# meudnaes/VoronoiRT

Measured on AMD Instinct MI355X. Metric: formal-solve cell-updates/sec, higher is better.
Workload: dtype f64

## Files before the change

### include/voronoirt.h

```cpp
#ifndef VORONOIRT_H
#define VORONOIRT_H

#include <stdint.h>

#ifdef __cplusplus
extern "C" {
#endif

#define VRT_OK 0
#define VRT_EINVAL (-1)
#define VRT_EGRID (-2)
#define VRT_ENODEVICE (-3)
#define VRT_ENOMEM (-4)
#define VRT_EIO (-5)

typedef struct vrt_grid vrt_grid;
typedef struct vrt_plan vrt_plan;

#define VRT_ALPHA_SITE 0
#define VRT_ALPHA_SITE_LAM 1
#define VRT_ALPHA_ANGLE_SITE_LAM 2
#define VRT_ALPHA_ANGLE_NATIVE 3
#define VRT_ALPHA_SITE_LAM_NATIVE 4

// ... 73 lines not shown
                                     double lambda0, double c0, const double *d_doppler_width, const double *d_gamma,
                                     double sigma_bb_const, const double *sigma_bf1, const double *sigma_bf2,
                                     const double *d_temperature, const double *d_lte_populations, double hc_over_kB,
                                     double pref_ij, double pref_ji, const double *d_C, const double *d_atom_density,
                                     double *d_R, double *d_populations, void *stream);
int vrt_lambda_update_native_dev_f32(vrt_plan *p, int64_t nlam, const float *dJ_up, const float *dJ_down,
                                     const float *dB_up, const double *deps, float *dS_up, float *dS_down,
                                     double *max_rel_change, void *stream);
int vrt_rates_populations_native_dev_f32(vrt_plan *p, int64_t nlam, const double *lambda, const int64_t blocks[6],
                                         const float *dJ_up, const float *dJ_down, const double *planck2,
                                         double lambda0, double c0, const double *d_doppler_width, const double *d_gamma,
                                         double sigma_bb_const, const double *sigma_bf1, const double *sigma_bf2,
                                         const double *d_temperature, const double *d_lte_populations, double hc_over_kB,
                                         double pref_ij, double pref_ji, const double *d_C, const double *d_atom_density,
                                         double *d_R, double *d_populations, void *stream);

int vrt_plan_execute_dev_f32(vrt_plan *p, int64_t nlam, int64_t ld, const float *dS,
                             const float *dalpha, int alpha_mode, const float *dI0_up,
                             const float *dI0_down, const double *weights_host, float *dJ,
                             float *dI_out, void *stream);
int vrt_plan_last_sweep_timing(const vrt_plan *p, double *ms, int64_t *launches);
int vrt_plan_patch_layout(const vrt_plan *p, int64_t *out);
int vrt_patch_dispatch_map(int order, int nrow, int nsplit, int lg_siblings, int64_t nred, int steps, int64_t *dims, int32_t *blocks);
int vrt_plan_patch_timeline(vrt_plan *p, int64_t cap_launches, int64_t cap_blocks, int64_t *launches, uint64_t *stamps, int64_t *counts);
int vrt_plan_check(vrt_plan *p);
int vrt_plan_last_path(const vrt_plan *p);
int vrt_plan_set_option(vrt_plan *p, const char *name, const char *value);
int vrt_grid_set_option(vrt_grid *g, const char *name, const char *value);

typedef struct vrt_schedule vrt_schedule;
int vrt_schedule_build(const vrt_grid *g, int dir, const int64_t *up, int n_sweeps, vrt_schedule **out);
int64_t vrt_schedule_num_nodes(const vrt_schedule *s);
int64_t vrt_schedule_num_levels(const vrt_schedule *s);
int vrt_schedule_get(const vrt_schedule *s, int64_t *site, int32_t *zflags, int64_t *level_off);
void vrt_schedule_destroy(vrt_schedule *s);
int vrt_layer_schedule(const vrt_grid *g, int dir, const int64_t *up, int n_sweeps, uint32_t *vis,
                       int32_t *nlev, int64_t *n_visits);
int vrt_layer_sorted_slots(const vrt_grid *g, int dir, const uint32_t *vis, int64_t *store, int64_t *self);

typedef struct vrt_patch_schedule vrt_patch_schedule;
int vrt_patch_schedule_build(const vrt_grid *g, int dir, const int64_t *up, int n_sweeps, int own_target,
                             int entry_cap, vrt_patch_schedule **out, int64_t counts[6]);
int vrt_patch_schedule_get(const vrt_patch_schedule *s, int32_t *layer_patch_off, int32_t *patch_own_lo,
                           int32_t *patch_own_cnt, int32_t *patch_nlev, int64_t *patch_ent_off,
                           int32_t *entry_pos, uint32_t *entry_vis, uint32_t *entry_loc);
int vrt_patch_schedule_get_deps(const vrt_patch_schedule *s, int64_t *dep_off, int32_t *dep_list);
// ... 248 lines not shown
```

### voronoirt_amd/_lib.py

```python
from __future__ import annotations

import ctypes
import os

HERE = os.path.dirname(os.path.abspath(__file__))
LIB_PATH = os.path.join(HERE, "libvrt_hip.so")
if os.environ.get("VRT_LIB_PATH"):
    LIB_PATH = os.environ["VRT_LIB_PATH"]

c_i64 = ctypes.c_int64
c_dbl = ctypes.c_double
p_i64 = ctypes.POINTER(ctypes.c_int64)
p_i32 = ctypes.POINTER(ctypes.c_int32)
p_dbl = ctypes.POINTER(ctypes.c_double)
p_int = ctypes.POINTER(ctypes.c_int)
vp = ctypes.c_void_p

VRT_OK, VRT_EINVAL, VRT_EGRID, VRT_ENODEVICE, VRT_ENOMEM, VRT_EIO = 0, -1, -2, -3, -4, -5
ALPHA_SITE, ALPHA_SITE_LAM, ALPHA_ANGLE_SITE_LAM, ALPHA_ANGLE_NATIVE, ALPHA_SITE_LAM_NATIVE = 0, 1, 2, 3, 4
METRIC_EUCLIDEAN, METRIC_PERIODIC_XY = 0, 1
RASTER_NEAREST, RASTER_INV_DIST2 = 1, 2
REG_FORMS = ("solve<256>", "solve<1024>", "xy_march_lds<1>", "xy_march_lds<2>", "xy_march_lds<4>", "xy_march_lds<0>",
             "xy_march_mem")
REG_FORM_KERNEL_MASK, REG_FORM_YZ_ROW_MARCH, REG_FORM_XZ_ROW_MARCH = 0xff, 0x100, 0x200
# ... 76 lines not shown
    "vrt_lambda_storage": (ctypes.c_int, [vp]),
    "vrt_lambda_iterate": (ctypes.c_int, [vp, p_dbl]),
    "vrt_lambda_get": (ctypes.c_int, [vp, p_dbl, p_dbl, p_dbl, p_dbl, p_dbl]),
    "vrt_lambda_destroy": (None, [vp]),
    "vrt_multi_create": (ctypes.c_int, [ctypes.c_int, p_int, c_i64, p_dbl, p_i64, c_i64, p_dbl, c_i64, p_dbl, p_int,
                                        ctypes.c_int, ctypes.POINTER(vp)]),
    "vrt_multi_execute": (ctypes.c_int, [vp, c_i64, c_i64, p_dbl, p_dbl, ctypes.c_int, p_dbl, p_dbl, p_dbl, p_dbl]),
    "vrt_multi_set_shard": (ctypes.c_int, [vp, ctypes.c_char_p]),
    "vrt_multi_last_shard": (ctypes.c_int, [vp]),
    "vrt_multi_uses_rccl": (ctypes.c_int, [vp]),
    "vrt_multi_destroy": (None, [vp]),
    "vrt_multi_execute_line": (ctypes.c_int, [vp, c_i64, c_i64, p_dbl, c_dbl, c_dbl, p_dbl, p_dbl, p_dbl, p_dbl, p_dbl, p_dbl,
                                              p_dbl, p_dbl, p_dbl, p_dbl]),
    "vrt_multi_lambda_create": (ctypes.c_int, [vp, ctypes.POINTER(LineCaseStruct), p_dbl, ctypes.POINTER(vp)]),
    "vrt_multi_lambda_iterate": (ctypes.c_int, [vp, p_dbl]),
    "vrt_multi_lambda_get": (ctypes.c_int, [vp, p_dbl, p_dbl, p_dbl, p_dbl, p_dbl]),
    "vrt_multi_lambda_destroy": (None, [vp]),
    "vrt_rates_populations_dev": (ctypes.c_int, [vp, c_i64, c_i64, p_dbl, p_i64, vp, p_dbl, c_dbl, c_dbl, vp, vp,
                                                 c_dbl, p_dbl, p_dbl, vp, vp, c_dbl, c_dbl, c_dbl, vp, vp, vp,
                                                 vp, vp]),
    "vrt_plan_last_sweep_timing": (ctypes.c_int, [vp, p_dbl, p_i64]),
    "vrt_plan_patch_layout": (ctypes.c_int, [vp, p_i64]),
    "vrt_patch_dispatch_map": (ctypes.c_int, [ctypes.c_int, ctypes.c_int, ctypes.c_int, ctypes.c_int, c_i64, ctypes.c_int, p_i64, p_i32]),
    "vrt_plan_patch_timeline": (ctypes.c_int, [vp, c_i64, c_i64, p_i64, ctypes.POINTER(ctypes.c_uint64), p_i64]),
    "vrt_plan_last_path": (ctypes.c_int, [vp]),
    "vrt_plan_set_option": (ctypes.c_int, [vp, ctypes.c_char_p, ctypes.c_char_p]),
    "vrt_grid_set_option": (ctypes.c_int, [vp, ctypes.c_char_p, ctypes.c_char_p]),
    "vrt_schedule_build": (ctypes.c_int, [vp, ctypes.c_int, p_i64, ctypes.c_int,
                                          ctypes.POINTER(vp)]),
    "vrt_schedule_num_nodes": (c_i64, [vp]),
    "vrt_schedule_num_levels": (c_i64, [vp]),
    "vrt_schedule_get": (ctypes.c_int, [vp, p_i64, p_i32, p_i64]),
    "vrt_schedule_destroy": (None, [vp]),
    "vrt_layer_schedule": (ctypes.c_int, [vp, ctypes.c_int, p_i64, ctypes.c_int,
                                          ctypes.POINTER(ctypes.c_uint32), p_i32, p_i64]),
    "vrt_layer_sorted_slots": (ctypes.c_int, [vp, ctypes.c_int, ctypes.POINTER(ctypes.c_uint32), p_i64, p_i64]),
    "vrt_patch_schedule_build": (ctypes.c_int, [vp, ctypes.c_int, p_i64, ctypes.c_int, ctypes.c_int, ctypes.c_int,
                                                ctypes.POINTER(vp), p_i64]),
    "vrt_patch_schedule_get": (ctypes.c_int, [vp, p_i32, p_i32, p_i32, p_i32, p_i64, p_i32,
                                              ctypes.POINTER(ctypes.c_uint32), ctypes.POINTER(ctypes.c_uint32)]),
    "vrt_patch_schedule_get_deps": (ctypes.c_int, [vp, p_i64, p_i32]),
    "vrt_patch_schedule_get_layers": (ctypes.c_int, [vp, ctypes.POINTER(ctypes.c_uint32), p_i32, p_i64]),
    "vrt_patch_schedule_destroy": (None, [vp]),
    "vrt_lambda_update_dev": (ctypes.c_int, [vp, c_i64, c_i64, vp, vp, vp, vp, vp, p_dbl, vp]),
    "vrt_short_characteristics": (ctypes.c_int, [c_i64, c_i64, c_i64, p_dbl, p_dbl, p_dbl, c_i64, p_dbl,
                                                 p_int, p_dbl, c_i64, p_dbl, c_i64, p_dbl, ctypes.c_int,
# ... 138 lines not shown
```

### voronoirt_amd/csrc/vrt_api.cpp

```cpp
#include <algorithm>
#include <atomic>
#include <chrono>
#include <cmath>
#include <cstdio>
#include <cstdlib>
#include <cstring>
#include <memory>
#include <new>
#include <thread>

#include "vrt_internal.h"

namespace vrt {

static thread_local std::string g_err;

void set_error(const std::string &msg) { g_err = msg; }
int fail(int code, const std::string &msg)
{
    g_err = msg;
    return code;
}

int check_source(const double *S, int64_t count)
// ... 6 lines not shown
int check_state_pointers(const void *session, const double *S, const double *populations)
{
    if (!session) return fail(VRT_EINVAL, "NULL session");
    if (!S && !populations) return fail(VRT_EINVAL, "S and populations are both NULL: nothing to set");
    return VRT_OK;
}

int check_state(int64_t n, int64_t nlam, const double *S, const double *populations)
{
    if (S)
        if (int rc = check_source(S, n * nlam)) return rc;
    if (populations)
        for (int64_t i = 0; i < 3 * n; i++)
            if (!std::isfinite(populations[i]) || !(populations[i] >= 0.0))
                return fail(VRT_EINVAL, "the populations must be finite and >= 0 everywhere");
    return VRT_OK;
}

void tuning_from_env(Tuning &t)
{
    static const char *names[] = {"VRT_PATH", "VRT_STEP_K", "VRT_STEP_SINGLE", "VRT_STEP_PAIRS", "VRT_STEP_XCD",
                                  "VRT_STEP_STREAMS", "VRT_STEP_LEVEL_MAP", "VRT_STEP_GROUP_DIR", "VRT_TILE_WIDE",
                                  "VRT_TILE_PRE", "VRT_PATCH_K", "VRT_PATCH_NT", "VRT_PATCH_OWN",
                                  "VRT_PATCH_Q", "VRT_PATCH_TARGET", "VRT_PATCH_SPLIT", "VRT_PATCH_ORDER", "VRT_PATCH_TIMELINE", "VRT_PAIR_BLOCK", "VRT_PATCH_QUAD", "VRT_PATCH_LEAN", "VRT_PATCH_CHAIN", "VRT_CHAIN_PAIRS", "VRT_CHAIN_SPIN", "VRT_CHAIN_DATAFLAG", "VRT_CHAIN_STATIC", "VRT_LAMBDA_NATIVE", "VRT_DEBUG_FLAGS", "VRT_DEBUG_SKIP_LEVELS",
                                  "VRT_TILE_DEBUG"};
    for (const char *nm : names) {
        const char *e = std::getenv(nm);
        if (e && *e && tuning_set(t, nm, e, false) != VRT_OK) {
            static std::mutex mu;
            static std::vector<std::string> said;
            std::lock_guard<std::mutex> lock(mu);
            if (std::find(said.begin(), said.end(), std::string(nm)) == said.end()) {
                said.push_back(nm);
                std::fprintf(stderr, "[libvrt_hip] ignoring %s=%s: %s\n", nm, e, g_err.c_str());
            }
        }
    }
}

int tuning_set(Tuning &t, const char *name, const char *value, bool created)
{
    if (!name || !value) return fail(VRT_EINVAL, "NULL option name or value");
    const std::string nm(name), v(value);
    if (nm == "VRT_PATH") {
        static const char *paths[] = {"auto", "levels", "tiles", "steps", "patches"};
        for (int i = 0; i < 5; i++)
            if (v == paths[i]) { t.path = i; return VRT_OK; }
        if (v.empty()) { t.path = 0; return VRT_OK; }
        return fail(VRT_EINVAL, "VRT_PATH must be auto, levels, tiles, steps or patches");
    }
    char *end = nullptr;
    const long x = std::strtol(value, &end, 10);
    if (end == value || *end != 0) return fail(VRT_EINVAL, "option " + nm + " needs an integer value");
    struct { const char *name; int *field; long lo, hi; bool creation_only; } tab[] = {
        {"VRT_STEP_K", &t.step_K, 0, 18, false}, {"VRT_STEP_SINGLE", &t.step_single, 0, 1, false},
        {"VRT_STEP_PAIRS", &t.step_pairs, 0, 64, false}, {"VRT_STEP_XCD", &t.step_xcd, 0, 2, false},
        {"VRT_STEP_STREAMS", &t.step_streams, 1, 4, false}, {"VRT_STEP_LEVEL_MAP", &t.step_level_map, 0, 1, false},
        {"VRT_STEP_GROUP_DIR", &t.step_group_dir, 0, 1, false}, {"VRT_TILE_WIDE", &t.tile_wide, 0, 1, false},
        {"VRT_TILE_PRE", &t.tile_pre, 0, 1, false},
        {"VRT_PATCH_K", &t.patch_K, 1, 8, true}, {"VRT_PATCH_NT", &t.patch_NT, 64, 1024, true},
        {"VRT_PATCH_OWN", &t.patch_own, 0, 65535, true}, {"VRT_PATCH_Q", &t.patch_Q, 1, 4, false},
        {"VRT_PATCH_TARGET", &t.patch_target, 0, 1 << 20, false}, {"VRT_PATCH_SPLIT", &t.patch_split, 0, 4096, false}, {"VRT_PATCH_ORDER", &t.patch_order, 0, 1, false},
        {"VRT_PATCH_TIMELINE", &t.patch_timeline, 0, 1, false}, {"VRT_PAIR_BLOCK", &t.pair_block, 1, 16, true},
        {"VRT_PATCH_QUAD", &t.patch_quad, 0, 1, true}, {"VRT_PATCH_LEAN", &t.patch_lean, 0, 1, false},
        {"VRT_PATCH_CHAIN", &t.patch_chain, 0, 2, false}, {"VRT_CHAIN_PAIRS", &t.chain_pairs, 1, 256, false},
        {"VRT_CHAIN_SPIN", &t.chain_spin, 1, 1 << 20, false}, {"VRT_CHAIN_DATAFLAG", &t.chain_dataflag, 0, 2, false},
        {"VRT_LAMBDA_NATIVE", &t.lambda_native, 0, 1, false}, {"VRT_CHAIN_STATIC", &t.chain_static, 0, 1, false}, {"VRT_DEBUG_FLAGS", &t.debug_flags, 0, 1 << 20, false},
        {"VRT_DEBUG_SKIP_LEVELS", &t.debug_skip_levels, 0, 1, false}, {"VRT_TILE_DEBUG", &t.tile_debug, 0, 1, false},
    };
    for (auto &o : tab)
        if (nm == o.name) {
            if (o.creation_only && created)
                return fail(VRT_EINVAL, "option " + nm + " shapes what plan creation builds: preset it in the environment");
            if (x < o.lo || x > o.hi) return fail(VRT_EINVAL, "option " + nm + " out of range");
            *o.field = (int)x;
            return VRT_OK;
        }
    return fail(VRT_EINVAL, "unknown option " + nm);
}

int use_device(int device)
{
    if (device < 0)
        return fail(VRT_ENODEVICE, "host-only grid handle (device < 0): no compute without a HIP device");
    int cnt = 0;
    hipError_t e = hipGetDeviceCount(&cnt);
    if (e != hipSuccess || cnt <= 0)
        return fail(VRT_ENODEVICE, "no HIP device available (libvrt_hip has no CPU fallback)");
    if (device < 0 || device >= cnt) return fail(VRT_EINVAL, "device ordinal out of range");
    VRT_HIP_TRY(hipSetDevice(device));
    (void)hipGetLastError();
    return VRT_OK;
// ... 1168 lines not shown
    const int maxL = p->tile_max_layers;
    int64_t fewest = 0;
    if (p->patch_ok && !p->h_patch_first.empty()) {
        fewest = INT64_MAX;
        for (int a = 0; a < p->A; a++)
            for (int layer = 2; layer <= maxL; layer++) {
                const int32_t *first = p->h_patch_first.data() + (size_t)a * (size_t)(maxL + 2);
                fewest = std::min<int64_t>(fewest, first[layer + 1] - first[layer]);
            }
        if (fewest == INT64_MAX) fewest = 0;
    }
    out[0] = p->patch_ok ? p->n_patches : 0;
    out[1] = fewest;
    out[2] = p->patch_work_off.empty() ? 0 : p->patch_work_off.back();
    out[3] = p->patch_work_padding;
    return VRT_OK;
}

int vrt_patch_dispatch_map(int order, int nrow, int nsplit, int lg_siblings, int64_t nred, int steps, int64_t *dims, int32_t *blocks)
{
    return guarded([&] { return patch_dispatch_map(order, nrow, nsplit, lg_siblings, nred, steps, dims, blocks); });
}

int vrt_plan_patch_timeline(vrt_plan *p, int64_t cap_launches, int64_t cap_blocks, int64_t *launches, uint64_t *stamps, int64_t *counts)
{
    if (!p || !launches || !stamps || !counts) return fail(VRT_EINVAL, "NULL plan or output");
    return guarded([&] {
        std::lock_guard<std::mutex> lock(p->mu);
        if (int rc = use_device(p->device)) return rc;
        return patch_timeline_read(p, cap_launches, cap_blocks, launches, stamps, counts);
    });
}

int vrt_plan_last_sweep_timing(const vrt_plan *p, double *ms, int64_t *launches)
{
    if (!p) return fail(VRT_EINVAL, "NULL plan");
    if (!p->ev_valid) return fail(VRT_EINVAL, "no execute has run on this plan yet");
    return guarded([&] {
        VRT_HIP_TRY(hipEventSynchronize(p->ev1));
        float t = 0.f;
        VRT_HIP_TRY(hipEventElapsedTime(&t, p->ev0, p->ev1));
        if (ms) *ms = (double)t;
        if (launches) *launches = p->last_launches;
        return patch_chain_check(const_cast<vrt_plan *>(p));
    });
}
// ... 304 lines not shown
```

### voronoirt_amd/csrc/vrt_device.h

```cpp
#pragma once

#include <hip/hip_runtime.h>

#include "vrt_internal.h"
#include "vrt_weights.h"

namespace vrt {

#ifdef VRT_DIAG
constexpr bool kDiag = true;
#else
constexpr bool kDiag = false;
#endif

constexpr uint32_t kNoSlot = 0xFFFFu;

__host__ __device__ __forceinline__ void pair_block_at(int q, int npair, int lgB, int &k0, int &lw)
{
    const int full = npair >> lgB << lgB;
    if (q < full) { k0 = q >> lgB << lgB; lw = lgB; return; }
    int k = full;
    const int r = npair - full;
    for (int bit = lgB - 1; bit >= 0; bit--)
        if (r & (1 << bit)) {
// ... 115 lines not shown
};

__device__ __forceinline__ double2 ld2(const double2 *base, unsigned idx)
{
    return *reinterpret_cast<const double2 *>(reinterpret_cast<const char *>(base) + ((size_t)idx << 4));
}
__device__ __forceinline__ double2 ld2(const float2 *base, unsigned idx)
{
    return to_d2(*reinterpret_cast<const float2 *>(reinterpret_cast<const char *>(base) + ((size_t)idx << 3)));
}

__device__ __forceinline__ void upwind_term(double r, double w, double a_c, double a_u, double S_c,
                                            double S_u, double I_u, bool early, bool inl, double &t,
                                            double &g, bool cheap = false)
{
    double ca, cb, ce;
    if (cheap) { ca = a_c; cb = a_u; ce = r; }
    else
    lin_weights(r * (a_c + a_u) / 2.0, ca, cb, ce);
    t = early ? ((ce * I_u + ca * S_u) + cb * S_c) * w : (ca * S_u + cb * S_c) * w;
    g = inl ? ce * w : 0.0;
}

struct PatchReduce {
    int nred = 0;
    int nblk[2] = {0, 0};
    int lo[2] = {0, 0}, hi[2] = {0, 0};
    int count[2] = {0, 0};
    int ppb = 4;
    void *Jd[2] = {nullptr, nullptr};
    double w[kMaxAngles];
    int32_t angles[2][kMaxAngles];
};


}
```

### voronoirt_amd/csrc/vrt_internal.h

```cpp
#pragma once

#include <hip/hip_runtime.h>

#include <algorithm>
#include <cstdint>
#include <memory>
#include <mutex>
#include <new>
#include <string>
#include <thread>
#include <vector>

#include "voronoirt.h"

namespace vrt {

void set_error(const std::string &msg);
int fail(int code, const std::string &msg);

int check_source(const double *S, int64_t count);
int check_state_pointers(const void *session, const double *S, const double *populations);
int check_state(int64_t n, int64_t nlam, const double *S, const double *populations);

#define VRT_HIP_TRY(expr)                                                                  \
// ... 155 lines not shown
        } catch (...) {
            threw[(size_t)t] = 1;
        }
    };
    std::vector<std::thread> pool;
    try {
        pool.reserve((size_t)std::max(count, 1));
    } catch (...) {
    }
    for (int t = 0; t < count; t++) {
        try {
            pool.emplace_back(guarded, t);
        } catch (...) {
            guarded(t);
        }
    }
    for (auto &th : pool) th.join();
    for (int t = 0; t < count; t++)
        if (threw[(size_t)t]) return false;
    return true;
}

constexpr int kMaxAngles = 64;
constexpr int64_t kMaxGuess = 70;
constexpr int32_t kNoUpwind = -1;

struct Direction {
    std::vector<int32_t> layer_of;
    std::vector<int64_t> perm;
    std::vector<int64_t> reduced;
    int64_t n1 = 0;
    DevBuf<int32_t> d_order;
    DevBuf<int32_t> d_rank;
    DevBuf<int32_t> d_lay;
    std::vector<int32_t> store;
    DevBuf<int32_t> d_store;
    DevBuf<int32_t> d_srank;
};

struct PlanCacheEntry;

struct CopyLane {
    Stream st;
    HostBuf<char> pin[2];
    Event ev[2];
};
// ... 4 lines not shown
    int step_K = 0;
    int step_single = 0;
    int step_pairs = 0;
    int step_xcd = 2;
    int step_streams = 2;
    int step_level_map = 1;
    int step_group_dir = 1;
    int tile_wide = 1;
    int tile_pre = 1;
    int patch_K = 1, patch_NT = 512;
    int patch_own = 0;
    int patch_Q = 1;
    int pair_block = 1;
    int patch_quad = 1;
    int patch_lean = 1;
    int patch_chain = 2;
    int chain_pairs = 9;
    int chain_spin = 2048;
    int chain_dataflag = 2;
    int patch_split = 0;
    int patch_target = 0;
    int patch_order = 1;
    int patch_timeline = 0;
    int chain_static = 1;
    int lambda_native = 1;
    int debug_flags = 0, debug_skip_levels = 0, tile_debug = 0;
};
void tuning_from_env(Tuning &t);
int tuning_set(Tuning &t, const char *name, const char *value, bool created);

struct ExecArgs {
    int64_t nlam = 0, ld = 0;
    const void *S = nullptr;
    const void *S_nat[2] = {nullptr, nullptr};
    const void *alpha = nullptr;
    int alpha_mode = 0;
    const void *I0[2] = {nullptr, nullptr};
    const double *weights = nullptr;
    void *J = nullptr;
    void *J_nat[2] = {nullptr, nullptr};
    void *I_out = nullptr;
    bool native = false;
    bool f32 = false;
    hipStream_t st = nullptr;
    bool wants_J() const { return native ? J_nat[0] != nullptr : J != nullptr; }
};
// ... 310 lines not shown
}
int alpha_to_native(vrt_plan *p, int64_t nlam, int64_t ld, const void *dalpha, void *out, hipStream_t st, bool f32);
int native_planes_ok(const vrt_plan *p, bool f32 = false);
int planes_to_native_f32(vrt_plan *p, int64_t nlam, int64_t ld, const float *din, float *out_up, float *out_down, hipStream_t st);
int plane_from_native_f32(vrt_plan *p, int dir_index, int64_t nlam, int64_t ld, const float *din, float *dout, hipStream_t st);
int J_from_native_f32(vrt_plan *p, int64_t nlam, int64_t ld, const float *dJ_up, const float *dJ_down, float *dJ, hipStream_t st);
int planes_to_native(vrt_plan *p, int64_t nlam, int64_t ld, const double *din, double *out_up, double *out_down, hipStream_t st);
int plane_from_native(vrt_plan *p, int dir_index, int64_t nlam, int64_t ld, const double *din, double *dout, hipStream_t st);
int J_from_native(vrt_plan *p, int64_t nlam, int64_t ld, const double *dJ_up, const double *dJ_down, double *dJ, hipStream_t st);
int execute_layers(vrt_plan *p, const ExecArgs &x, int path);
int64_t steps_max_layer(bool f32);

struct TileArgs;
struct PatchReduce;
bool patch_shape_exists(int K, int Q, int NT);
int launch_patch_entries(vrt_plan *p, int a, int64_t first, int64_t count);
int ensure_patch_work(vrt_plan *p, int G, const std::vector<int32_t> &group_angles, const std::vector<int> &group_off);
int launch_patch_layer(vrt_plan *p, const TileArgs &ta, int npair, int layer, int group, int Q, hipStream_t st,
                       bool f32, const PatchReduce *reduce);
constexpr int kPatchTimelineRec = 12;
void patch_timeline_begin(vrt_plan *p);
int patch_timeline_read(vrt_plan *p, int64_t cap_launches, int64_t cap_blocks, int64_t *launches, uint64_t *stamps, int64_t *counts);
int patch_dispatch_map(int order, int nrow, int nsplit, int lg_siblings, int64_t nred, int steps, int64_t *dims, int32_t *blocks);
bool patch_chain_possible(const vrt_plan *p, int npair, bool f32);
bool patch_chain_dataflag(const vrt_plan *p, int npair, bool f32);
int launch_patch_chain(vrt_plan *p, const TileArgs &ta, int npair, hipStream_t st, bool f32, const PatchReduce *reduce,
                       bool dataflag, bool ctrl_zeroed = false);
int chain_ctrl_words();
int patch_chain_check(vrt_plan *p);

struct NgRange {
    int64_t dense = 0, tail = 0, tstride = 1;
};
struct NgState {
    int order = 0, start = 0, period = 0;
    DevBuf<double> hist[3];
    unsigned have = 0;
    DevBuf<double> d_ws;
    int last_applied = 0;
    double last_sums[5] = {0, 0, 0, 0, 0}, last_coeffs[2] = {0, 0};
};
inline NgRange ng_S_range(int64_t n, int64_t nlam, bool sweep_order)
{
    NgRange rg;
    if (sweep_order) { rg.dense = (nlam / 2) * 2 * n; rg.tail = nlam & 1 ? n : 0; rg.tstride = 2; }
    else { rg.dense = (n * nlam) & ~(int64_t)1; rg.tail = (n * nlam) & 1; rg.tstride = 1; }
// ... 54 lines not shown
```

### voronoirt_amd/csrc/vrt_patch.hip

```cpp
#include <hip/hip_runtime.h>

#include <algorithm>
#include <cmath>
#include <cstdio>
#include <cstdlib>
#include <cstring>
#include <type_traits>

#include "vrt_device.h"
#include "vrt_internal.h"

namespace vrt {

enum : int {
    kDiagNoLevels = 1, kDiagCentreGathers = 2, kDiagNoWeights = 4, kDiagNoStores = 8, kDiagNoGatherI = 16, kDiagNoGatherAlpha = 32,
    kDiagNoGatherS = 64, kDiagNoReduce = 128, kDiagNoWait = 256, kDiagPlainLoadI = 512, kDiagPlainStoreI = 1024, kDiagNoPairLoop = 2048,
    kDiagDirectTable = 4096,
};
__host__ __device__ __forceinline__ constexpr bool diag(int dbg, int flag) { return kDiag && (dbg & flag) != 0; }

struct PatchArgs {
    TileArgs ta;
    int npair;
    int layer;
    int ngrp;
    int nrow;
    int order;
    int prow;
    unsigned row_rcp;
    int nsplit, Q;
    int sbase, srem;
    int lgB;
    int stride;
    int cap;
    int quad;
    int lean;
    int dbg_ent0, dbg_ent_stride, dbg_ent_last;
    int dbg;
    unsigned long long *tl;
    PatchReduce red;
    const int4 *wrec;
    const int32_t *e_pos, *e_u1, *e_u2;
    const uint32_t *e_vis, *e_loc;
    const double *e_w1, *e_w2, *e_r1, *e_r2;
};

__global__ void __launch_bounds__(256)
k_patch_entries(int64_t count, const int32_t *__restrict__ e_pos, const int32_t *__restrict__ t_u1,
                const int32_t *__restrict__ t_u2, const double *__restrict__ t_w1, const double *__restrict__ t_w2,
                const double *__restrict__ t_r1, const double *__restrict__ t_r2, int32_t *__restrict__ e_u1,
                int32_t *__restrict__ e_u2, double *__restrict__ e_w1, double *__restrict__ e_w2,
                double *__restrict__ e_r1, double *__restrict__ e_r2)
{
    const int64_t e = (int64_t)blockIdx.x * blockDim.x + threadIdx.x;
    if (e >= count) return;
    const int p = e_pos[e];
    e_u1[e] = t_u1[p]; e_u2[e] = t_u2[p];
    e_w1[e] = t_w1[p]; e_w2[e] = t_w2[p];
    e_r1[e] = t_r1[p]; e_r2[e] = t_r2[p];
}

int launch_patch_entries(vrt_plan *p, int a, int64_t first, int64_t count)
{
// ... 97 lines not shown
    {
        if (kDiag && pa.tl) {
            slot = pa.tl + 3 * ((size_t)blockIdx.y * gridDim.x + blockIdx.x);
            t0 = wall_clock64();
        }
    }
    __device__ __forceinline__ void steps(const PatchArgs &pa, int b0, int b1)
    {
        if (kDiag) share = (unsigned long long)((b1 - b0 + pa.Q - 1) / pa.Q);
    }
    __device__ __forceinline__ void reduces()
    {
        if (kDiag) share = 1ull << 32;
    }
    __device__ __forceinline__ ~BlockStamp()
    {
        if (kDiag && slot && threadIdx.x == 0) {
            slot[0] = t0;
            slot[1] = wall_clock64();
            slot[2] = share;
        }
    }
};
template <typename T, int NT>
__device__ __forceinline__ void patch_reduce_role(const PatchArgs &pa)
{
    typedef typename Pair<T>::type T2;
    const TileArgs &ta = pa.ta;
    const int tid = threadIdx.x;
    int b = reduce_block_index(pa), r = 0;
    if (b >= pa.red.nblk[0]) { b -= pa.red.nblk[0]; r = 1; }
    if (b >= pa.red.nblk[r]) return;
    if (diag(pa.dbg, kDiagNoReduce)) return;
    const int len = pa.red.hi[r] - pa.red.lo[r];
    const int per = NT * pa.red.ppb;
    const int nblock = pair_block_count(pa.npair, pa.lgB);
    int k0 = 0, lw = 0;
    for (int k = 0; k < nblock; k++) {
        pair_block_of(k, pa.npair, pa.lgB, k0, lw);
        const int cnt = (int)((((int64_t)len << lw) + per - 1) / per);
        if (b < cnt) break;
        b -= cnt;
    }
    const int64_t nn = ta.n;
    const size_t run = (size_t)len << lw;
    const size_t base = (size_t)k0 * (size_t)nn + ((size_t)pa.red.lo[r] << lw);
    T2 *Jd = reinterpret_cast<T2 *>(pa.red.Jd[r]);
    const T2 *I0 = reinterpret_cast<const T2 *>(ta.I);
    const size_t plane = (size_t)pa.npair * (size_t)nn;
    if (pa.red.ppb == 4) {
        const size_t f0 = (size_t)b * 4 * NT + tid;
        const unsigned left = f0 < run ? (unsigned)min((size_t)(run - f0 + NT - 1) / NT, (size_t)4) : 0u;
        const size_t e0 = base + (left ? f0 : 0);
        double ax[4], ay[4];
#pragma unroll
        for (int i = 0; i < 4; i++) { ax[i] = 0.0; ay[i] = 0.0; }
        for (int j = 0; j < pa.red.count[r]; j++) {
            const int a = pa.red.angles[r][j];
            const T2 *Ia = I0 + (size_t)a * plane + e0;
            double2 v[4];
#pragma unroll
            for (int i = 0; i < 4; i++) v[i] = to_d2(Ia[(unsigned)i < left ? i * NT : 0]);
#pragma unroll
            for (int i = 0; i < 4; i++) {
                ax[i] += pa.red.w[a] * v[i].x;
                ay[i] += pa.red.w[a] * v[i].y;
            }
        }
#pragma unroll
        for (int i = 0; i < 4; i++)
            if ((unsigned)i < left) Jd[e0 + (size_t)i * NT] = from_d2<T>(make_double2(ax[i], ay[i]));
        return;
    }
    for (int i = 0; i < pa.red.ppb; i++) {
        const size_t f = ((size_t)b * pa.red.ppb + i) * NT + tid;
        if (f >= run) break;
        const size_t e = base + f;
        double ax = 0.0, ay = 0.0;
        for (int j = 0; j < pa.red.count[r]; j++) {
            const int a = pa.red.angles[r][j];
            const double2 v = to_d2(I0[(size_t)a * plane + e]);
            ax += pa.red.w[a] * v.x;
            ay += pa.red.w[a] * v.y;
        }
        Jd[e] = from_d2<T>(make_double2(ax, ay));
    }
}

#ifdef VRT_PATCH_WPE
#define VRT_WPE_ATTR __attribute__((amdgpu_waves_per_eu(VRT_PATCH_WPE, VRT_PATCH_WPE)))
#else
#define VRT_WPE_ATTR
#endif
template <typename T, int AM, int K, int Q, int NT>
__global__ void __launch_bounds__(NT) VRT_WPE_ATTR
k_patch_solve(PatchArgs pa)
{
    typedef typename Pair<T>::type T2;
    extern __shared__ __attribute__((aligned(16))) double2 ptile[];
    const TileArgs &ta = pa.ta;
    const int tid = threadIdx.x;
    BlockStamp stamp(pa);
    if (reduce_block_index(pa) >= 0) {
        stamp.reduces();
        patch_reduce_role<T, NT>(pa);
        return;
    }
    const PatchBlock blk = patch_block(pa, pa.lgB);
    const int x = blk.lane, sj = blk.row;
// ... 746 lines not shown
    __syncthreads();
    quad_pairs<AM, NT, false>(pair_io<AM>(pa, it.d), it, tab, ptile);
}


struct ChainDev {
    TileArgs ta;
    int npair, nsplit, cap;
    const int32_t *e_pos, *e_u1, *e_u2;
    const uint32_t *e_vis, *e_loc;
    const double *e_w1, *e_w2, *e_r1, *e_r2;
    PatchReduce red;
    const int4 *items;
    int q_off[9];
    const int32_t *deps;
    uint32_t *progress;
    uint32_t *ctrl;
    uint32_t *host_status;
    int64_t n_patches;
    uint32_t spin_limit;
    int static_items;
    int dbg;
};

__device__ __forceinline__ const uint32_t *chain_abort_word(const uint32_t *cd_words)
{
    return reinterpret_cast<const ChainDev *>(cd_words)->ctrl + kChainAbortWord;
}

__device__ __forceinline__ int cd_int(const int *p) { return __builtin_amdgcn_readfirstlane(*p); }
template <typename P>
__device__ __forceinline__ P *cd_ptr(P *const *p) { return uniform_ptr(*p); }

__device__ __forceinline__ void chain_wait_slow(const int32_t *s_dep, int step)
{
    const int lane = (int)(threadIdx.x & 63u);
    const uint32_t *ctl = reinterpret_cast<const uint32_t *>(s_dep - kCtlWords);
    const ChainDev *cd = reinterpret_cast<const ChainDev *>(((uint64_t)ctl[kCtlArgsHi] << 32) | (uint64_t)ctl[kCtlArgsLo]);
    uint32_t *abort_word = cd->ctrl + kChainAbortWord;
    const uint32_t *progress = chain_progress(ctl);
    const uint32_t target = ctl[kCtlBase] + (uint32_t)step, limit = cd->spin_limit;
    const int ndep = (int)ctl[kCtlNdep];
    for (int c0 = 0; c0 < ndep; c0 += 64) {
        const int j = c0 + lane;
        const int dep = j < 64 + kChainDepLds ? s_dep[j] : (j < ndep ? (cd->deps + ctl[kCtlDepOff])[j] : (int)ctl[kCtlSelf]);
        const uint32_t *w = progress + dep;
// ... 271 lines not shown
            const size_t base = work.size();
            work.resize(base + slots * 8 * 2, make_int4(0, 0, 0, 0));
            p->patch_work_padding += (int64_t)(slots * 8 - m);
            for (int x = 0; x < 8; x++) {
                const size_t b0 = m * (size_t)x / 8, b1 = m * (size_t)(x + 1) / 8;
                for (size_t t = b0; t < b1; t++) {
                    const int32_t q = items[t].second;
                    const int2 r2 = p->h_patch_rec2[(size_t)q];
                    const int d = p->dir_of_active[(size_t)r2.y] > 0 ? 0 : 1;
                    const Direction &dir = d == 0 ? p->g->up : p->g->down;
                    const size_t slot = base + 2 * ((t - b0) * 8 + (size_t)x);
                    work[slot] = p->h_patch_rec[(size_t)q];
                    work[slot + 1] = make_int4(r2.x, r2.y | (d << 16), (int)(dir.reduced[(size_t)layer - 1] - 1), (int)(dir.reduced[(size_t)layer] - 1));
                }
            }
        }
    p->patch_work_off.back() = (int64_t)(work.size() / 2);
    if (int rc = p->d_patch_work.alloc(work.size())) return rc;
    VRT_HIP_TRY(hipMemcpy(p->d_patch_work, work.data(), sizeof(int4) * work.size(), hipMemcpyHostToDevice));
    p->patch_work_groups = G;
    return VRT_OK;
}

static void size_reduce(PatchReduce &red, int npair, int lgB, int NT)
{
    red.nred = 0;
    int64_t total = 0;
    for (int r = 0; r < 2; r++)
        if (red.count[r] > 0 && red.Jd[r]) total += (int64_t)std::max(0, red.hi[r] - red.lo[r]) * npair;
    red.ppb = total <= (int64_t)NT * 1024 ? 1 : 4;
    const int64_t per = (int64_t)NT * red.ppb;
    const int nblock = pair_block_count(npair, lgB);
    for (int r = 0; r < 2; r++) {
        const int64_t len = red.hi[r] - red.lo[r];
        red.nblk[r] = 0;
        if (len > 0 && red.count[r] > 0 && red.Jd[r])
            for (int k = 0; k < nblock; k++) {
                int k0, lw;
                pair_block_of(k, npair, lgB, k0, lw);
                red.nblk[r] += (int)(((len << lw) + per - 1) / per);
            }
        red.nred += red.nblk[r];
    }
    red.nred = (red.nred + 7) / 8 * 8;
}

int launch_patch_layer(vrt_plan *p, const TileArgs &ta, int npair, int layer, int group, int Q, hipStream_t st,
                       bool f32, const PatchReduce *reduce)
{
    const int target_wgs = p->tune.patch_target;
    const int maxL = p->tile_max_layers;
    const size_t wo = (size_t)group * (size_t)(maxL + 2) + (size_t)layer;
    const int64_t w0 = (layer >= 2 && layer <= maxL) ? p->patch_work_off[wo] : 0, w1 = (layer >= 2 && layer <= maxL) ? p->patch_work_off[wo + 1] : 0;
    PatchArgs pa;
    if (reduce) {
        pa.red = *reduce;
        size_reduce(pa.red, npair, native_lg(p, f32), p->patch_NT);
    }
    if (w1 <= w0 && pa.red.nred == 0) return VRT_OK;
    pa.ta = ta;
    pa.npair = npair;
    pa.layer = layer;
    pa.lgB = native_lg(p, f32);
    pa.quad = (f32 && pa.lgB >= 1 && p->patch_K == 1 && p->tune.patch_quad != 0 && (npair & 1) == 0) ? 1 : 0;
    if (pa.quad) Q = 1;
    pa.lean = (p->tune.patch_lean != 0 && p->patch_K == 1 && Q == 1 && !pa.quad && npair >= 2) ? 1 : 0;
    const int lgS = pa.lgB - pa.quad;
    pa.Q = Q;
    pa.nsplit = 1;
    pa.ngrp = 1 << lgS;
    if (w1 > w0) {
        const int64_t items = (w1 - w0) << lgS;
        const int nblock = pair_block_count(npair, pa.lgB);
        const int steps_all = (nblock + Q - 1) / Q;
        int nsplit;
        if (p->tune.patch_split > 0) nsplit = std::min(steps_all, p->tune.patch_split);
        else if (target_wgs > 0) nsplit = (int)std::max<int64_t>(1, std::min<int64_t>(steps_all, (target_wgs + items - 1) / items));
        else {
            const double T = std::min(900.0, 460.0 + 4100.0 / (double)steps_all);
            const int s_min = (int)std::min<int64_t>(steps_all, std::max<int64_t>(1, (512 + items - 1) / items));
// ... 415 lines not shown
```

Before: 90.30 billion.

## Restructure patch angle-reduction with O(1) block map and batched multi-angle loads

Replaces the per-block linear search over pair blocks with a precomputed reduce map that uses a reciprocal divide to find each block's pair group and offset. The reduction loop now issues loads for several angles at once, up to a fixed depth, using scalar base pointers before accumulating. Angles and weights are packed into a compact per-range array, so the kernel no longer indexes a weight table by angle. It also adds tunable ppb and depth options and a host query for the block map. The risks are higher register pressure from the batched loads and larger kernel arguments.

```diff
diff --git a/include/voronoirt.h b/include/voronoirt.h
--- a/include/voronoirt.h
+++ b/include/voronoirt.h
@@ -119,6 +119,7 @@
 int vrt_plan_last_sweep_timing(const vrt_plan *p, double *ms, int64_t *launches);
 int vrt_plan_patch_layout(const vrt_plan *p, int64_t *out);
 int vrt_patch_dispatch_map(int order, int nrow, int nsplit, int lg_siblings, int64_t nred, int steps, int64_t *dims, int32_t *blocks);
+int vrt_patch_reduce_map(const int64_t *len, const int *count, int npair, int lg_block, int nt, int ppb, int64_t *dims, int32_t *blocks);
 int vrt_plan_patch_timeline(vrt_plan *p, int64_t cap_launches, int64_t cap_blocks, int64_t *launches, uint64_t *stamps, int64_t *counts);
 int vrt_plan_check(vrt_plan *p);
 int vrt_plan_last_path(const vrt_plan *p);
diff --git a/voronoirt_amd/_lib.py b/voronoirt_amd/_lib.py
--- a/voronoirt_amd/_lib.py
+++ b/voronoirt_amd/_lib.py
@@ -122,6 +122,7 @@
     "vrt_plan_last_sweep_timing": (ctypes.c_int, [vp, p_dbl, p_i64]),
     "vrt_plan_patch_layout": (ctypes.c_int, [vp, p_i64]),
     "vrt_patch_dispatch_map": (ctypes.c_int, [ctypes.c_int, ctypes.c_int, ctypes.c_int, ctypes.c_int, c_i64, ctypes.c_int, p_i64, p_i32]),
+    "vrt_patch_reduce_map": (ctypes.c_int, [p_i64, p_i32, ctypes.c_int, ctypes.c_int, ctypes.c_int, ctypes.c_int, p_i64, p_i32]),
     "vrt_plan_patch_timeline": (ctypes.c_int, [vp, c_i64, c_i64, p_i64, ctypes.POINTER(ctypes.c_uint64), p_i64]),
     "vrt_plan_last_path": (ctypes.c_int, [vp]),
     "vrt_plan_set_option": (ctypes.c_int, [vp, ctypes.c_char_p, ctypes.c_char_p]),
diff --git a/voronoirt_amd/csrc/vrt_api.cpp b/voronoirt_amd/csrc/vrt_api.cpp
--- a/voronoirt_amd/csrc/vrt_api.cpp
+++ b/voronoirt_amd/csrc/vrt_api.cpp
@@ -52,7 +52,7 @@
     static const char *names[] = {"VRT_PATH", "VRT_STEP_K", "VRT_STEP_SINGLE", "VRT_STEP_PAIRS", "VRT_STEP_XCD",
                                   "VRT_STEP_STREAMS", "VRT_STEP_LEVEL_MAP", "VRT_STEP_GROUP_DIR", "VRT_TILE_WIDE",
                                   "VRT_TILE_PRE", "VRT_PATCH_K", "VRT_PATCH_NT", "VRT_PATCH_OWN",
-                                  "VRT_PATCH_Q", "VRT_PATCH_TARGET", "VRT_PATCH_SPLIT", "VRT_PATCH_ORDER", "VRT_PATCH_TIMELINE", "VRT_PAIR_BLOCK", "VRT_PATCH_QUAD", "VRT_PATCH_LEAN", "VRT_PATCH_CHAIN", "VRT_CHAIN_PAIRS", "VRT_CHAIN_SPIN", "VRT_CHAIN_DATAFLAG", "VRT_CHAIN_STATIC", "VRT_LAMBDA_NATIVE", "VRT_DEBUG_FLAGS", "VRT_DEBUG_SKIP_LEVELS",
+                                  "VRT_PATCH_Q", "VRT_PATCH_TARGET", "VRT_PATCH_SPLIT", "VRT_PATCH_ORDER", "VRT_PATCH_TIMELINE", "VRT_PATCH_REDUCE_PPB", "VRT_PATCH_REDUCE_DEPTH", "VRT_PAIR_BLOCK", "VRT_PATCH_QUAD", "VRT_PATCH_LEAN", "VRT_PATCH_CHAIN", "VRT_CHAIN_PAIRS", "VRT_CHAIN_SPIN", "VRT_CHAIN_DATAFLAG", "VRT_CHAIN_STATIC", "VRT_LAMBDA_NATIVE", "VRT_DEBUG_FLAGS", "VRT_DEBUG_SKIP_LEVELS",
                                   "VRT_TILE_DEBUG"};
     for (const char *nm : names) {
         const char *e = std::getenv(nm);
@@ -92,12 +92,14 @@
         {"VRT_PATCH_OWN", &t.patch_own, 0, 65535, true}, {"VRT_PATCH_Q", &t.patch_Q, 1, 4, false},
         {"VRT_PATCH_TARGET", &t.patch_target, 0, 1 << 20, false}, {"VRT_PATCH_SPLIT", &t.patch_split, 0, 4096, false}, {"VRT_PATCH_ORDER", &t.patch_order, 0, 1, false},
         {"VRT_PATCH_TIMELINE", &t.patch_timeline, 0, 1, false}, {"VRT_PAIR_BLOCK", &t.pair_block, 1, 16, true},
+        {"VRT_PATCH_REDUCE_PPB", &t.patch_reduce_ppb, 0, 4, false}, {"VRT_PATCH_REDUCE_DEPTH", &t.patch_reduce_depth, 0, kReduceDepth, false},
         {"VRT_PATCH_QUAD", &t.patch_quad, 0, 1, true}, {"VRT_PATCH_LEAN", &t.patch_lean, 0, 1, false},
         {"VRT_PATCH_CHAIN", &t.patch_chain, 0, 2, false}, {"VRT_CHAIN_PAIRS", &t.chain_pairs, 1, 256, false},
         {"VRT_CHAIN_SPIN", &t.chain_spin, 1, 1 << 20, false}, {"VRT_CHAIN_DATAFLAG", &t.chain_dataflag, 0, 2, false},
         {"VRT_LAMBDA_NATIVE", &t.lambda_native, 0, 1, false}, {"VRT_CHAIN_STATIC", &t.chain_static, 0, 1, false}, {"VRT_DEBUG_FLAGS", &t.debug_flags, 0, 1 << 20, false},
         {"VRT_DEBUG_SKIP_LEVELS", &t.debug_skip_levels, 0, 1, false}, {"VRT_TILE_DEBUG", &t.tile_debug, 0, 1, false},
     };
+    if (nm == "VRT_PATCH_REDUCE_PPB" && x == 3) return fail(VRT_EINVAL, "option VRT_PATCH_REDUCE_PPB must be 0, 1, 2 or 4");
     for (auto &o : tab)
         if (nm == o.name) {
             if (o.creation_only && created)
@@ -1312,6 +1314,11 @@
     return guarded([&] { return patch_dispatch_map(order, nrow, nsplit, lg_siblings, nred, steps, dims, blocks); });
 }
 
+int vrt_patch_reduce_map(const int64_t *len, const int *count, int npair, int lg_block, int nt, int ppb, int64_t *dims, int32_t *blocks)
+{
+    return guarded([&] { return patch_reduce_map(len, count, npair, lg_block, nt, ppb, dims, blocks); });
+}
+
 int vrt_plan_patch_timeline(vrt_plan *p, int64_t cap_launches, int64_t cap_blocks, int64_t *launches, uint64_t *stamps, int64_t *counts)
 {
     if (!p || !launches || !stamps || !counts) return fail(VRT_EINVAL, "NULL plan or output");
diff --git a/voronoirt_amd/csrc/vrt_device.h b/voronoirt_amd/csrc/vrt_device.h
--- a/voronoirt_amd/csrc/vrt_device.h
+++ b/voronoirt_amd/csrc/vrt_device.h
@@ -161,6 +161,60 @@
     g = inl ? ce * w : 0.0;
 }
 
+constexpr int kReduceTails = 4;
+struct ReduceMap {
+    int full = 0;
+    int cfull = 1;
+    unsigned rcp = 0xFFFFFFFFu;
+    int tail[kReduceTails] = {0, 0, 0, 0};
+};
+struct ReduceBlock { int k0, lw, bb; };
+__host__ inline int64_t reduce_map_fill(ReduceMap &m, int64_t len, int npair, int lgB, int64_t per)
+{
+    m = ReduceMap();
+    if (len <= 0 || npair <= 0) return 0;
+    const int nfull = npair >> lgB;
+    const int64_t cfull = ((len << lgB) + per - 1) / per;
+    int64_t total = (int64_t)nfull * cfull;
+    m.cfull = (int)cfull;
+    m.full = (int)total;
+    m.rcp = cfull <= 1 ? 0xFFFFFFFFu : (unsigned)(((uint64_t)1 << 32) / (uint64_t)cfull);
+    const int rem = npair - (nfull << lgB);
+    int t = 0;
+    for (int bit = lgB - 1; bit >= 0; bit--)
+        if (rem & (1 << bit)) {
+            const int64_t c = ((len << bit) + per - 1) / per;
+            m.tail[t++] = (int)c;
+            total += c;
+        }
+    return total;
+}
+__host__ __device__ __forceinline__ ReduceBlock reduce_block_of(const ReduceMap &m, int npair, int lgB, unsigned b)
+{
+    ReduceBlock o;
+    if (b < (unsigned)m.full) {
+        unsigned k = (unsigned)(((unsigned long long)b * m.rcp) >> 32);
+        unsigned bb = b - k * (unsigned)m.cfull;
+        if (bb >= (unsigned)m.cfull) { k++; bb -= (unsigned)m.cfull; }
+        o.k0 = (int)(k << lgB); o.lw = lgB; o.bb = (int)bb;
+        return o;
+    }
+    b -= (unsigned)m.full;
+    o.k0 = npair >> lgB << lgB;
+    o.lw = 0;
+    const int rem = npair - o.k0;
+    int t = 0;
+    for (int bit = lgB - 1; bit >= 0; bit--)
+        if (rem & (1 << bit)) {
+            o.lw = bit;
+            if (b < (unsigned)m.tail[t]) break;
+            b -= (unsigned)m.tail[t++];
+            o.k0 += 1 << bit;
+        }
+    o.bb = (int)b;
+    return o;
+}
+
 struct PatchReduce {
     int nred = 0;
     int nblk[2] = {0, 0};
@@ -171,6 +225,19 @@
     double w[kMaxAngles];
     int32_t angles[2][kMaxAngles];
 };
-
-
-}
+struct PatchReduceArgs {
+    int nred = 0;
+    int nblk[2] = {0, 0};
+    int lo[2] = {0, 0}, hi[2] = {0, 0};
+    int count[2] = {0, 0};
+    int first[2] = {0, 0};
+    int ppb = 4;
+    int depth = 0;
+    ReduceMap map[2];
+    void *Jd[2] = {nullptr, nullptr};
+    double ws[kMaxAngles + kReduceDepth];
+    int32_t angles[kMaxAngles + kReduceDepth];
+};
+
+
+}
diff --git a/voronoirt_amd/csrc/vrt_internal.h b/voronoirt_amd/csrc/vrt_internal.h
--- a/voronoirt_amd/csrc/vrt_internal.h
+++ b/voronoirt_amd/csrc/vrt_internal.h
@@ -201,6 +201,7 @@
 }
 
 constexpr int kMaxAngles = 64;
+constexpr int kReduceDepth = 10;
 constexpr int64_t kMaxGuess = 70;
 constexpr int32_t kNoUpwind = -1;
 
@@ -251,6 +252,8 @@
     int patch_target = 0;
     int patch_order = 1;
     int patch_timeline = 0;
+    int patch_reduce_ppb = 0;
+    int patch_reduce_depth = 0;
     int chain_static = 1;
     int lambda_native = 1;
     int debug_flags = 0, debug_skip_levels = 0, tile_debug = 0;
@@ -607,6 +610,7 @@
 void patch_timeline_begin(vrt_plan *p);
 int patch_timeline_read(vrt_plan *p, int64_t cap_launches, int64_t cap_blocks, int64_t *launches, uint64_t *stamps, int64_t *counts);
 int patch_dispatch_map(int order, int nrow, int nsplit, int lg_siblings, int64_t nred, int steps, int64_t *dims, int32_t *blocks);
+int patch_reduce_map(const int64_t *len, const int *count, int npair, int lgB, int NT, int ppb, int64_t *dims, int32_t *blocks);
 bool patch_chain_possible(const vrt_plan *p, int npair, bool f32);
 bool patch_chain_dataflag(const vrt_plan *p, int npair, bool f32);
 int launch_patch_chain(vrt_plan *p, const TileArgs &ta, int npair, hipStream_t st, bool f32, const PatchReduce *reduce,
diff --git a/voronoirt_amd/csrc/vrt_patch.hip b/voronoirt_amd/csrc/vrt_patch.hip
--- a/voronoirt_amd/csrc/vrt_patch.hip
+++ b/voronoirt_amd/csrc/vrt_patch.hip
@@ -38,7 +38,7 @@
     int dbg_ent0, dbg_ent_stride, dbg_ent_last;
     int dbg;
     unsigned long long *tl;
-    PatchReduce red;
+    PatchReduceArgs red;
     const int4 *wrec;
     const int32_t *e_pos, *e_u1, *e_u2;
     const uint32_t *e_vis, *e_loc;
@@ -182,69 +182,91 @@
         }
     }
 };
+template <typename T> struct ReduceLoads { static constexpr int value = sizeof(T) == 8 ? 10 : 16; };
+template <typename T2> struct RawPair;
+template <> struct RawPair<double2> { typedef double type __attribute__((ext_vector_type(2))); };
+template <> struct RawPair<float2> { typedef float type __attribute__((ext_vector_type(2))); };
+typedef const __attribute__((address_space(1))) char *GlobalBytes;
+__device__ __forceinline__ GlobalBytes scalar_base(const void *p)
+{
+    unsigned lo = (unsigned)(uint64_t)p, hi = (unsigned)((uint64_t)p >> 32);
+    asm("" : "+s"(lo), "+s"(hi));
+    return (GlobalBytes)(((uint64_t)hi << 32) | (uint64_t)lo);
+}
+template <typename T, int NT, int E>
+__device__ __forceinline__ void patch_reduce_sum(const PatchReduceArgs &red, int r, const typename Pair<T>::type *I0, size_t plane,
+                                                 typename Pair<T>::type *Jd, size_t e0, unsigned left)
+{
+    typedef typename Pair<T>::type T2;
+    typedef typename RawPair<T2>::type Raw;
+    constexpr int D = ReduceLoads<T>::value / E < kReduceDepth ? ReduceLoads<T>::value / E : kReduceDepth;
+    constexpr int lg = Log2Size<T2>::value;
+    const unsigned t0 = left ? threadIdx.x : 0u;
+    unsigned off[E];
+#pragma unroll
+    for (int i = 0; i < E; i++) off[i] = (t0 + ((unsigned)i < left ? (unsigned)(i * NT) : 0u)) << lg;
+    double ax[E], ay[E];
+#pragma unroll
+    for (int i = 0; i < E; i++) { ax[i] = 0.0; ay[i] = 0.0; }
+    const int count = red.count[r], first = red.first[r];
+    const int dep = red.depth > 0 && red.depth < D ? red.depth : D;
+    for (int j0 = 0; j0 < count; j0 += dep) {
+        int aj[D];
+        double wj[D];
+#pragma unroll
+        for (int j = 0; j < D; j++) { aj[j] = red.angles[first + j0 + j]; wj[j] = red.ws[first + j0 + j]; }
+        const int m = min(dep, count - j0);
+        Raw v[D][E];
+#pragma unroll
+        for (int j = 0; j < D; j++)
+            if (j < m) {
+                const GlobalBytes pl = scalar_base(I0 + (size_t)aj[j] * plane + e0);
+#pragma unroll
+                for (int i = 0; i < E; i++) {
+                    unsigned o = off[i];
+                    asm volatile("" : "+v"(o));
+                    v[j][i] = *reinterpret_cast<const __attribute__((address_space(1))) Raw *>(pl + o);
+                }
+            }
+#pragma unroll
+        for (int j = 0; j < D; j++)
+            if (j < m) {
+#pragma unroll
+                for (int i = 0; i < E; i++) {
+                    ax[i] += wj[j] * (double)v[j][i].x;
+                    ay[i] += wj[j] * (double)v[j][i].y;
+                }
+            }
+    }
+#pragma unroll
+    for (int i = 0; i < E; i++)
+        if ((unsigned)i < left) Jd[e0 + t0 + (size_t)(i * NT)] = from_d2<T>(make_double2(ax[i], ay[i]));
+}
+
 template <typename T, int NT>
 __device__ __forceinline__ void patch_reduce_role(const PatchArgs &pa)
 {
     typedef typename Pair<T>::type T2;
     const TileArgs &ta = pa.ta;
-    const int tid = threadIdx.x;
     int b = reduce_block_index(pa), r = 0;
     if (b >= pa.red.nblk[0]) { b -= pa.red.nblk[0]; r = 1; }
     if (b >= pa.red.nblk[r]) return;
     if (diag(pa.dbg, kDiagNoReduce)) return;
+    const ReduceBlock rb = reduce_block_of(pa.red.map[r], pa.npair, pa.lgB, (unsigned)b);
     const int len = pa.red.hi[r] - pa.red.lo[r];
-    const int per = NT * pa.red.ppb;
-    const int nblock = pair_block_count(pa.npair, pa.lgB);
-    int k0 = 0, lw = 0;
-    for (int k = 0; k < nblock; k++) {
-        pair_block_of(k, pa.npair, pa.lgB, k0, lw);
-        const int cnt = (int)((((int64_t)len << lw) + per - 1) / per);
-        if (b < cnt) break;
-        b -= cnt;
-    }
+    const int ppb = pa.red.ppb;
     const int64_t nn = ta.n;
-    const size_t run = (size_t)len << lw;
-    const size_t base = (size_t)k0 * (size_t)nn + ((size_t)pa.red.lo[r] << lw);
+    const size_t run = (size_t)len << rb.lw;
+    const size_t f0 = (size_t)rb.bb * (size_t)(NT * ppb);
+    const size_t e0 = (size_t)rb.k0 * (size_t)nn + ((size_t)pa.red.lo[r] << rb.lw) + f0;
+    const size_t mine = f0 + threadIdx.x;
+    const unsigned left = mine < run ? (unsigned)min((size_t)(run - mine + NT - 1) / NT, (size_t)ppb) : 0u;
     T2 *Jd = reinterpret_cast<T2 *>(pa.red.Jd[r]);
     const T2 *I0 = reinterpret_cast<const T2 *>(ta.I);
     const size_t plane = (size_t)pa.npair * (size_t)nn;
-    if (pa.red.ppb == 4) {
-        const size_t f0 = (size_t)b * 4 * NT + tid;
-        const unsigned left = f0 < run ? (unsigned)min((size_t)(run - f0 + NT - 1) / NT, (size_t)4) : 0u;
-        const size_t e0 = base + (left ? f0 : 0);
-        double ax[4], ay[4];
-#pragma unroll
-        for (int i = 0; i < 4; i++) { ax[i] = 0.0; ay[i] = 0.0; }
-        for (int j = 0; j < pa.red.count[r]; j++) {
-            const int a = pa.red.angles[r][j];
-            const T2 *Ia = I0 + (size_t)a * plane + e0;
-            double2 v[4];
-#pragma unroll
-            for (int i = 0; i < 4; i++) v[i] = to_d2(Ia[(unsigned)i < left ? i * NT : 0]);
-#pragma unroll
-            for (int i = 0; i < 4; i++) {
-                ax[i] += pa.red.w[a] * v[i].x;
-                ay[i] += pa.red.w[a] * v[i].y;
-            }
-        }
-#pragma unroll
-        for (int i = 0; i < 4; i++)
-            if ((unsigned)i < left) Jd[e0 + (size_t)i * NT] = from_d2<T>(make_double2(ax[i], ay[i]));
-        return;
-    }
-    for (int i = 0; i < pa.red.ppb; i++) {
-        const size_t f = ((size_t)b * pa.red.ppb + i) * NT + tid;
-        if (f >= run) break;
-        const size_t e = base + f;
-        double ax = 0.0, ay = 0.0;
-        for (int j = 0; j < pa.red.count[r]; j++) {
-            const int a = pa.red.angles[r][j];
-            const double2 v = to_d2(I0[(size_t)a * plane + e]);
-            ax += pa.red.w[a] * v.x;
-            ay += pa.red.w[a] * v.y;
-        }
-        Jd[e] = from_d2<T>(make_double2(ax, ay));
-    }
+    if (ppb == 4) patch_reduce_sum<T, NT, 4>(pa.red, r, I0, plane, Jd, e0, left);
+    else if (ppb == 2) patch_reduce_sum<T, NT, 2>(pa.red, r, I0, plane, Jd, e0, left);
+    else patch_reduce_sum<T, NT, 1>(pa.red, r, I0, plane, Jd, e0, left);
 }
 
 #ifdef VRT_PATCH_WPE
@@ -1037,6 +1059,7 @@
     int static_items;
     int dbg;
 };
+static_assert(sizeof(PatchArgs) <= 4096 && sizeof(ChainDev) <= 4096, "kernel arguments: 4 KiB at most");
 
 __device__ __forceinline__ const uint32_t *chain_abort_word(const uint32_t *cd_words)
 {
@@ -1354,27 +1377,63 @@
     return VRT_OK;
 }
 
-static void size_reduce(PatchReduce &red, int npair, int lgB, int NT)
-{
-    red.nred = 0;
+static int size_reduce(PatchReduceArgs &red, const PatchReduce &req, int npair, int lgB, int NT, int ppb_opt, int depth)
+{
+    red = PatchReduceArgs();
     int64_t total = 0;
     for (int r = 0; r < 2; r++)
-        if (red.count[r] > 0 && red.Jd[r]) total += (int64_t)std::max(0, red.hi[r] - red.lo[r]) * npair;
-    red.ppb = total <= (int64_t)NT * 1024 ? 1 : 4;
+        if (req.count[r] > 0 && req.Jd[r]) total += (int64_t)std::max(0, req.hi[r] - req.lo[r]) * npair;
+    red.ppb = ppb_opt == 1 || ppb_opt == 2 || ppb_opt == 4 ? ppb_opt : (total <= (int64_t)NT * 1024 ? 1 : 4);
+    red.depth = depth;
     const int64_t per = (int64_t)NT * red.ppb;
-    const int nblock = pair_block_count(npair, lgB);
+    int64_t nred = 0;
+    int used = 0;
     for (int r = 0; r < 2; r++) {
-        const int64_t len = red.hi[r] - red.lo[r];
-        red.nblk[r] = 0;
-        if (len > 0 && red.count[r] > 0 && red.Jd[r])
-            for (int k = 0; k < nblock; k++) {
-                int k0, lw;
-                pair_block_of(k, npair, lgB, k0, lw);
-                red.nblk[r] += (int)(((len << lw) + per - 1) / per);
-            }
-        red.nred += red.nblk[r];
-    }
-    red.nred = (red.nred + 7) / 8 * 8;
+        const int64_t len = req.hi[r] - req.lo[r];
+        const bool any = len > 0 && req.count[r] > 0 && req.Jd[r];
+        red.lo[r] = req.lo[r]; red.hi[r] = req.hi[r]; red.Jd[r] = req.Jd[r];
+        red.count[r] = any ? req.count[r] : 0;
+        red.first[r] = used;
+        if (used + red.count[r] > kMaxAngles) return fail(VRT_EINVAL, "the two ranges of a reduction hold more angles than a plan may have");
+        const int64_t nb = reduce_map_fill(red.map[r], any ? len : 0, npair, lgB, per);
+        red.nblk[r] = (int)std::min<int64_t>(nb, INT32_MAX / 4);
+        nred += red.nblk[r];
+        for (int j = 0; j < red.count[r]; j++) {
+            red.angles[used + j] = req.angles[r][j];
+            red.ws[used + j] = req.w[req.angles[r][j]];
+        }
+        used += red.count[r];
+    }
+    red.nred = (int)((nred + 7) / 8 * 8);
+    return VRT_OK;
+}
+
+int patch_reduce_map(const int64_t *len, const int *count, int npair, int lgB, int NT, int ppb, int64_t *dims, int32_t *blocks)
+{
+    if (!len || !count || !dims) return fail(VRT_EINVAL, "NULL argument");
+    if (npair < 1 || lgB < 0 || lgB > kReduceTails || NT < 64 || NT > 1024 || ppb < 0 || ppb > 4 || ppb == 3 || len[0] < 0 || len[1] < 0 ||
+        len[0] >= ((int64_t)1 << 28) || len[1] >= ((int64_t)1 << 28) || count[0] < 0 || count[1] < 0 || count[0] > kMaxAngles || count[1] > kMaxAngles)
+        return fail(VRT_EINVAL, "reduce map: argument out of range");
+    PatchReduce red{};
+    static double plane_stub;
+    for (int r = 0; r < 2; r++) {
+        red.lo[r] = 0; red.hi[r] = (int)len[r];
+        red.count[r] = count[r];
+        red.Jd[r] = &plane_stub;
+    }
+    PatchReduceArgs ra;
+    if (int rc = size_reduce(ra, red, npair, lgB, NT, ppb, 0)) return rc;
+    dims[0] = ra.nred; dims[1] = ra.nblk[0]; dims[2] = ra.nblk[1]; dims[3] = ra.ppb;
+    if (!blocks) return VRT_OK;
+    for (int i = 0; i < ra.nred; i++) {
+        int32_t *o = blocks + 4 * (size_t)i;
+        int b = i, r = 0;
+        if (b >= ra.nblk[0]) { b -= ra.nblk[0]; r = 1; }
+        if (b >= ra.nblk[r]) { o[0] = -1; o[1] = o[2] = o[3] = 0; continue; }
+        const ReduceBlock rb = reduce_block_of(ra.map[r], npair, lgB, (unsigned)b);
+        o[0] = r; o[1] = rb.k0; o[2] = rb.lw; o[3] = rb.bb;
+    }
+    return VRT_OK;
 }
 
 int launch_patch_layer(vrt_plan *p, const TileArgs &ta, int npair, int layer, int group, int Q, hipStream_t st,
@@ -1386,8 +1445,7 @@
     const int64_t w0 = (layer >= 2 && layer <= maxL) ? p->patch_work_off[wo] : 0, w1 = (layer >= 2 && layer <= maxL) ? p->patch_work_off[wo + 1] : 0;
     PatchArgs pa;
     if (reduce) {
-        pa.red = *reduce;
-        size_reduce(pa.red, npair, native_lg(p, f32), p->patch_NT);
+        if (int rc = size_reduce(pa.red, *reduce, npair, native_lg(p, f32), p->patch_NT, p->tune.patch_reduce_ppb, p->tune.patch_reduce_depth)) return rc;
     }
     if (w1 <= w0 && pa.red.nred == 0) return VRT_OK;
     pa.ta = ta;
```

After: 92.84 billion (median of 6 runs). +2.8%, better.
